# ScuffleCloud/SVT-AV1-mirror

Measured on AMD Instinct MI355X. Metric: open-loop ME 64x64 superblocks/sec + achieved HBM GB/s, 4K preset-8, higher is better.
Workload: dtype u8

## Files before the change

### svt-av1-mirror_amd/csrc/svtme_stages.hip

```cpp
#include <hip/hip_ext.h>
#include <cstdlib>
#include <type_traits>

#include "svtme_me_common.h"

extern "C" bool svtme_hme_rt(const svtme_controls *c);

namespace svtme {


#define STAGE_A_BUF_DW 1024
#define STAGE_B_BUF_DW 640

template <int ND, typename P>
__device__ __forceinline__ void rows_qsad(P rp, int bstride_dw, const uint8_t *src, int src_stride,
                                          int k0, int k1, uint32_t acc[4]) {
    constexpr int CH = 64 / ND;
    for (int kc = k0; kc < k1; kc += CH) {
        const int ke         = min(k1, kc + CH);
        unsigned long long a = 0;
#pragma unroll 2
        for (int k = kc; k < ke; k++) {
            const P rd         = rp + k * bstride_dw;
            const uint32_t *sd = (const uint32_t *)(src + k * src_stride);
// ... 2265 lines not shown
        const uint32_t d3 = __builtin_amdgcn_alignbyte(t5, t4.w, (uint32_t)sh);
#pragma unroll
        for (int j = 0; j < NT; j++) {
            const int r = k - j;
            if (r < 0 || r >= ROWS)
                continue;
            acc[j][0] = qsad64(pair(d0, d1), src[r][0], acc[j][0]);
            acc[j][0] = qsad64(pair(d1, d2), src[r][1], acc[j][0]);
            acc[j][1] = qsad64(pair(d1, d2), src[r][0], acc[j][1]);
            acc[j][1] = qsad64(pair(d2, d3), src[r][1], acc[j][1]);
        }
    }
#pragma unroll
    for (int j = 0; j < NT; j++)
        M.template add_quads<true>((uint32_t)acc[j][0], (uint32_t)(acc[j][0] >> 32), (uint32_t)acc[j][1],
                                   (uint32_t)(acc[j][1] >> 32), obase + (uint32_t)((c + NC * j) * 8), 0, 8, qb);
}

template <bool SUB>
__device__ __forceinline__ void fp_rows32_whole(PuMin<true> &M, const uint8_t *g, int sdw, int h, uint32_t obase,
                                                const uint32_t (&src)[SUB ? 4 : 8][2], int by, int bx) {
    g     = uni_ptr(g);
    sdw   = UNI(sdw);
    h     = UNI(h);
    obase = (uint32_t)UNI(obase);
    const uint32_t qb = PuMin<true>::quad_b_rows();
    const int sh      = (int)((uintptr_t)g & 3);
    const __amdgpu_buffer_rsrc_t rs = plane_rsrc(g - sh);
    const uint32_t lo = (uint32_t)((by * 8) * sdw + bx * 2) * 4u;
    if constexpr (SUB) {
        fp_whole_class<true, 2>(M, rs, lo, sdw, sh, qb, obase, 0, src);
        if (h == 4)
            fp_whole_class<true, 2>(M, rs, lo, sdw, sh, qb, obase, 1, src);
        else
            fp_whole_class<true, 1>(M, rs, lo, sdw, sh, qb, obase, 1, src);
    } else {
        fp_whole_class<false, 4>(M, rs, lo, sdw, sh, qb, obase, 0, src);
        fp_whole_class<false, 4>(M, rs, lo, sdw, sh, qb, obase, 4, src);
    }
}

template <bool SUB>
__device__ __forceinline__ uint32_t fp_probe32(PuMin<true> &M, const uint8_t *g, int sdw,
                                               const uint32_t (&src)[SUB ? 4 : 8][2], int by, int bx) {
    constexpr int ROWS = SUB ? 4 : 8, RSTEP = SUB ? 2 : 1;
    g         = uni_ptr(g);
    sdw       = UNI(sdw);
    const int sh = (int)((uintptr_t)g & 3);
    const __amdgpu_buffer_rsrc_t rs = plane_rsrc(g - sh);
    const uint32_t lo = (uint32_t)((by * 8) * sdw + bx * 2) * 4u;
    u32x4a4 d[ROWS];
#pragma unroll
    for (int rr = 0; rr < ROWS; rr++) d[rr] = bld4(rs, lo, (uint32_t)(rr * RSTEP * sdw) * 4u);
    uint32_t s8 = 0;
#pragma unroll
    for (int rr = 0; rr < ROWS; rr++) {
        s8 = __builtin_amdgcn_sad_u8(__builtin_amdgcn_alignbyte(d[rr].y, d[rr].x, (uint32_t)sh), src[rr][0], s8);
        s8 = __builtin_amdgcn_sad_u8(__builtin_amdgcn_alignbyte(d[rr].z, d[rr].y, (uint32_t)sh), src[rr][1], s8);
    }
    M.add_probe(s8);
    return SUB ? s8 << 1 : s8;
}

struct FpArea {
    int16_t xo, yo, w, h, xc, yc;
    bool probe;
};
template <typename Probe>
__device__ __forceinline__ FpArea fp_area(const DevJob &dj, const SbGeo &G, int s, uint32_t zz, uint32_t rdiv,
                                          int16_t sc_x, int16_t sc_y, Probe probe_var) {
    const svtme_job &job    = dj.job;
    const svtme_controls &c = job.ctrl;
    const int l = s >> 2, r = s & 3;
    const uint32_t ox = G.ox, oy = G.oy;
    const bool mctf   = SF(job, me_type) == SVTME_ME_MCTF;
    const DevPlane &C = dj.cur.lv[0];
    const DevPlane &P = dj.ref[l][r].lv[0];
    int16_t xc = sc_x, yc = sc_y;
    uint16_t dist = ref_dist_const(job, l, r);
    if (!mctf)
        dist = scaled_dist(dist);
    int16_t w = i16(min((int)(SF(c, me_sa.sa_min.width) * dist), (int)SF(c, me_sa.sa_max.width)));
    int16_t h = i16(min((int)(SF(c, me_sa.sa_min.height) * dist), (int)SF(c, me_sa.sa_max.height)));
    if (SF(c, mv_sa_adj_enabled) && (!SF(c, mv_sa_adj_nearest_ref_only) || r == 0)) {
        const int mth = (int)SF(c, mv_sa_adj_mv_size_th), mul = (int)SF(c, mv_sa_adj_sa_multiplier);
        if (absi(xc) > mth)
            w = i16(w * mul);
        if (absi(yc) > mth)
            h = i16(h * mul);
    }
    w = i16((max(1u, ((uint32_t)(int32_t)w / rdiv)) + 7) & ~0x07u);
    h = i16(max(3u, ((uint32_t)(int32_t)h / rdiv)));
    const int16_t pad = 63, org_x = (int16_t)ox, org_y = (int16_t)oy;
    if (c.me_early_exit_th) {
        if (zz < (c.me_early_exit_th / 6)) {
            w = 1;
            h = 1;
        }
    } else if ((xc != 0 || yc != 0) && SF(job, is_ref)) {
        const int16_t pw = i16(P.width), ph = i16(P.height);
        xc = ((org_x + xc) < -pad) ? i16(-pad - org_x) : xc;
        xc = ((org_x + xc) > pw - 1) ? i16(xc - ((org_x + xc) - (pw - 1))) : xc;
        yc = ((org_y + yc) < -pad) ? i16(-pad - org_y) : yc;
        yc = ((org_y + yc) > ph - 1) ? i16(yc - ((org_y + yc) - (ph - 1))) : yc;
        const uint8_t *cb = C.base + (ptrdiff_t)oy * C.stride + ox;
        const uint32_t zero_sad =
            wave_nxm(P.base + (ptrdiff_t)oy * P.stride + ox, 2 * P.stride, cb, 2 * C.stride, (int)(G.bh >> 1),
                     (int)G.bw)
            << 1;
        const uint32_t hme_mv_sad = wave_nxm(P.base + (ptrdiff_t)((int)oy + yc) * P.stride + ((int)ox + xc),
                                             2 * P.stride, cb, 2 * C.stride, (int)(G.bh >> 1), (int)G.bw)
            << 1;
        const uint64_t zc = (uint64_t)zero_sad << 8, hc = (uint64_t)hme_mv_sad << 8;
        if (min_u64(zc, hc) == zc) {
            xc = 0;
            yc = 0;
        }
    }
    const bool probe = SF(c, me_8x8_var_enabled) && (w * h > 24);
    if (probe) {
        const uint32_t var = probe_var(P.base + (ptrdiff_t)((int)oy + yc) * P.stride + ((int)ox + xc));
        if (var > c.me_sr_mult2_th) {
            w = i16((max(1, w * 3 / 2) + 7) & ~0x7);
            h = i16(max(1, h * 3 / 2));
        }
        if (var < c.me_sr_div4_th) {
            w = i16((max(1, w >> 2) + 7) & ~0x7);
            h = i16(max(1, h >> 2));
            h = i16(max(3, (int)h));
        } else if (var < c.me_sr_div2_th) {
            w = i16((min((int)w, w >> 1) + 7) & ~0x7);
            h = i16(min((int)h, h >> 1));
            h = i16(max(3, (int)h));
        }
    }
    const int16_t pic_w = (int16_t)job.width, pic_h = (int16_t)job.height;
    int16_t xo = i16(xc - (w >> 1));
    int16_t yo = i16(yc - (h >> 1));
    xo = ((org_x + xo) < -pad) ? i16(-pad - org_x) : xo;
    w  = ((org_x + xo) < -pad) ? i16(w - (-pad - (org_x + xo))) : w;
    xo = ((org_x + xo) > pic_w - 1) ? i16(xo - ((org_x + xo) - (pic_w - 1))) : xo;
    w  = ((org_x + xo + w) > pic_w) ? i16(max(1, w - ((org_x + xo + w) - pic_w))) : w;
    w  = (w < 8) ? w : i16(w & ~0x07);
    yo = ((org_y + yo) < -pad) ? i16(-pad - org_y) : yo;
    h  = ((org_y + yo) < -pad) ? i16(h - (-pad - (org_y + yo))) : h;
    yo = ((org_y + yo) > pic_h - 1) ? i16(yo - ((org_y + yo) - (pic_h - 1))) : yo;
    h  = (org_y + yo + h > pic_h) ? i16(max(1, h - ((org_y + yo + h) - pic_h))) : h;
    return FpArea{xo, yo, w, h, xc, yc, probe};
}

__device__ __forceinline__ bool direct_records(const DevJob &dj) {
    return SF(dj.job, me_type) == SVTME_ME_MCTF && dj.parts == 1 && dj.out_sb == nullptr;
}
__device__ __forceinline__ void direct_record(svtme_ref_record *rec, const CSlot &v, unsigned long long k8,
                                              unsigned long long k16, unsigned long long k32, unsigned long long k64) {
    const int lane   = threadIdx.x & 63;
    uint32_t *o      = (uint32_t *)rec;
    const uint32_t wm = magic_u32((uint32_t)max(1, (int)v.w));
    auto put = [&](unsigned long long key, int pu) {
        uint32_t sad = U32MAX, mv = 0;
        if (v.searched) {
            const uint32_t ord = (uint32_t)key;
            sad                = (uint32_t)(key >> 32);
            int16_t mx, my;
            if (v.probe && ord == 0) {
                mx = v.xc;
                my = v.yc;
            } else {
                const int p = (int)ord - (int)v.probe;
                const int q = mdiv(p, wm);
                my          = i16(v.yo + q);
                mx          = i16(v.xo + (p - q * v.w));
            }
            mv = ((uint32_t)(uint16_t)my << 16) | (uint16_t)mx;
        }
        o[pu]      = sad;
        o[85 + pu] = mv;
    };
    put(k8, 21 + lane);
    if ((lane & 3) == 0)
        put(k16, 5 + (lane >> 2));
    if ((lane & 15) == 0)
        put(k32, 1 + (lane >> 4));
    if (lane == 63)
        put(k64, 0);
    if (lane < 6) {
        const uint32_t t[6] = {(uint32_t)v.hme_sad, (uint32_t)(v.hme_sad >> 32),
                               (uint32_t)(uint16_t)v.sc_x | ((uint32_t)(uint16_t)v.sc_y << 16), v.zz,
                               (uint32_t)v.searched | ((uint32_t)v.do_ref << 8) | ((uint32_t)v.tf_exit << 16), 0u};
        o[170 + lane] = t[lane];
    }
}

__device__ __forceinline__ CSlot fp_unsearched(uint64_t hme_sad, uint32_t zz, int16_t sc_x, int16_t sc_y, uint8_t dref,
                                               uint8_t tf_exit) {
    return CSlot{hme_sad, zz, sc_x, sc_y, 0, 0, 0, 0, 0, 0, dref, 0, tf_exit};
}

template <bool SUB, bool K32, int TQ = (SUB ? FP_TQ : 2), bool WIDE = false, int WHOLE = 7>
__device__ __forceinline__ void fp_slot(const DevJob &dj, const SbGeo &G, int s, const uint32_t (&src)[SUB ? 4 : 8][2],
                                        int by, int bx, uint64_t hme_sad, uint32_t zz, uint32_t rdiv, int16_t sc_x,
                                        int16_t sc_y, uint8_t dref, uint8_t tf_exit, int part, uint32_t parts,
                                        unsigned long long *kp, CSlot *cs, svtme_ref_record *rec = nullptr) {
    const int lane = threadIdx.x & 63;
    const int l = s >> 2, r = s & 3;
    const uint32_t ox = G.ox, oy = G.oy;
    if (!dref || tf_exit) {
        const CSlot cv = fp_unsearched(hme_sad, zz, sc_x, sc_y, dref, tf_exit);
        if (part == 0 && lane == 0)
            *cs = cv;
        if (rec)
            direct_record(rec, cv, 0, 0, 0, 0);
        return;
    }
    const DevPlane &P = dj.ref[l][r].lv[0];
    PuMin<K32> M;
    M.clear();
    const FpArea A = fp_area(dj, G, s, zz, rdiv, sc_x, sc_y, [&](const uint8_t *g) {
        const int sh = (int)((uintptr_t)g & 3);
        uint32_t p8, p64;
        if constexpr (K32) {
            p8  = fp_probe32<SUB>(M, g, P.stride >> 2, src, by, bx);
            p64 = wave_sum_u32(p8);
        } else {
            fp_rows<SUB, K32, 1>(M, (const uint32_t *)(g - sh), P.stride >> 2, sh, 1, 1, 0, 1, 0u, src, by, bx);
            M.finalize();
            p8  = (uint32_t)(PuMin<K32>::template out<SUB>(M.b8, true) >> 32);
            p64 = rl32((uint32_t)(PuMin<K32>::template out<SUB>(M.b64, false) >> 32), 63);
        }
        const uint32_t mean = p64 / 64;
        const int32_t diff  = (int32_t)p8 - (int32_t)mean;
        return wave_sum_u32((uint32_t)(diff * diff)) / 64;
    });
    const int16_t xo = A.xo, yo = A.yo, w = A.w, h = A.h, xc = A.xc, yc = A.yc;
    const bool probe = A.probe;
    HME_SUB(22);

    const uint8_t *g = P.base + (ptrdiff_t)((int)oy + yo) * P.stride + ((int)ox + xo);
    const int sh     = (int)((uintptr_t)g & 3);
    const int nq     = (sh + w + 3) >> 2;
    const int y0 = (int)(((uint32_t)h * part) / parts), y1 = (int)(((uint32_t)h * (part + 1)) / parts);
    const uint32_t obase = probe ? 1u : 0u;
    if constexpr (K32) {
        const bool whole = !WIDE && w == 8 && parts == 1;
        if ((SUB ? (WHOLE & 2) && (h == 3 || h == 4) : (WHOLE & 1) && h == 8) && whole)
            fp_rows32_whole<SUB>(M, g, P.stride >> 2, h, obase, src, by, bx);
        else
            fp_rows32<SUB, WIDE ? 6 : 2>(M, g, P.stride >> 2, w, y0, y1, obase, src, by, bx);
    }
    else
        fp_rows<SUB, K32, TQ>(M, (const uint32_t *)(g - sh), P.stride >> 2, sh, w, nq, y0, y1, obase, src, by, bx);
    HME_SUB(23);
    M.finalize();
    const unsigned long long k8  = PuMin<K32>::template out<SUB>(M.b8, true);
    const unsigned long long k16 = PuMin<K32>::template out<SUB>(M.b16, false);
    const unsigned long long k32 = PuMin<K32>::template out<SUB>(M.b32, false);
    const unsigned long long k64 = PuMin<K32>::template out<SUB>(M.b64, false);
    if (parts == 1) {
        kp[21 + lane] = k8;
        if ((lane & 3) == 0)
            kp[5 + (lane >> 2)] = k16;
        if ((lane & 15) == 0)
            kp[1 + (lane >> 4)] = k32;
        if (lane == 63)
            kp[0] = k64;
    } else {
        atomicMin(&kp[21 + lane], k8);
        if ((lane & 3) == 0)
            atomicMin(&kp[5 + (lane >> 2)], k16);
        if ((lane & 15) == 0)
            atomicMin(&kp[1 + (lane >> 4)], k32);
        if (lane == 63)
            atomicMin(&kp[0], k64);
    }
    const CSlot cv{hme_sad, zz, sc_x, sc_y, xo, yo, w, xc, yc, 1, dref, (uint8_t)probe, 0};
    if (part == 0 && lane == 0)
        *cs = cv;
    if (rec)
        direct_record(rec, cv, k8, k16, k32, k64);
}


template <bool SUB, bool K32, bool WIDE = false>
__global__ void __launch_bounds__(256) __attribute__((amdgpu_waves_per_eu(SUB ? 5 : 4, 8))) k_stage_c1(const DevBatch B) {
    const int lane = threadIdx.x & 63, wid = threadIdx.x >> 6;
    const uint32_t u = UNI(xcd_remap(blockIdx.x, gridDim.x) * 4 + wid);
    if (u >= B.total)
        return;
    uint32_t gw;
    const DevJob &dj        = batch_job(B, u, &gw);
    const svtme_job &job    = dj.job;
    const uint32_t parts  = dj.parts;
    const uint32_t per_sb = dj.R * parts;
    const uint32_t sb_local = UNI(gw / per_sb);
    const uint32_t rem      = gw - sb_local * per_sb;
    const int k             = UNI(rem / parts);
    const int part          = UNI(rem - (uint32_t)k * parts);
    const int s             = k < job.num_refs[0] ? k : 4 + (k - job.num_refs[0]);
    const SbGeo G     = sb_geo(dj, sb_local);
    const uint32_t ox = G.ox, oy = G.oy;
    const bool mctf   = job.me_type == SVTME_ME_MCTF;
    constexpr int ROWS = SUB ? 4 : 8, RSTEP = SUB ? 2 : 1;
    const int z16 = lane >> 2, k4 = lane & 3;
    const int by  = ((z16 >> 3) << 2) | (((z16 >> 1) & 1) << 1) | (k4 >> 1);
    const int bx  = (((z16 >> 2) & 1) << 2) | ((z16 & 1) << 1) | (k4 & 1);

    const DevPlane &C = dj.cur.lv[0];
    uint32_t src[ROWS][2];
#pragma unroll
    for (int rr = 0; rr < ROWS; rr++) {
        const uint32_t *sp =
            (const uint32_t *)(C.base + (ptrdiff_t)(oy + by * 8 + rr * RSTEP) * C.stride + ox + bx * 8);
        src[rr][0] = sp[0];
        src[rr][1] = sp[1];
    }
    const SlotCentre scv   = final_centre(job, dj.bst + sb_local, valid_mask(job));
    const uint64_t hme_sad = rl64(scv.hme_sad, s);
    const uint32_t zz = rl32(scv.zz, s), rdiv = rl32(scv.reduce_div, s);
    const int16_t sc_x = (int16_t)rl32((uint32_t)(int32_t)scv.sc_x, s);
    const int16_t sc_y = (int16_t)rl32((uint32_t)(int32_t)scv.sc_y, s);
    const uint8_t dref = (uint8_t)rl32(scv.do_ref, s);
    const uint8_t tf_exit = mctf && rl64(scv.hme_sad, 0) < job.tf_me_exit_th;
    CSlot *cs = dj.cslot + (size_t)sb_local * dj.R + k;
    unsigned long long *kp = dj.keys + ((size_t)sb_local * dj.R + k) * SVTME_PU_COUNT;
    svtme_ref_record *rec = direct_records(dj) ? dj.out_records + (size_t)sb_local * dj.R + k : nullptr;
    fp_slot<SUB, K32, (SUB ? FP_TQ : 2), WIDE>(dj, G, s, src, by, bx, hme_sad, zz, rdiv, sc_x, sc_y, dref, tf_exit, part,
                                             parts, kp, cs, rec);
}

#define FPW_PITCH 80
#define FPW_BOFF 40
#define FPW_ROWS 96
#define FPW_TQ 4

struct FpW {
    uint32_t b8t, b8b, b16, b32, b64;
};

__device__ __forceinline__ uint32_t fpw_min_hr(uint32_t v) {
    return min_u32(v, (uint32_t)__builtin_amdgcn_update_dpp((int)v, (int)v, 0x128, 0xF, 0xF, false));
}

template <bool MASK, bool K8 = true>
__device__ __forceinline__ void fpw_pair(FpW &m, unsigned long long T, unsigned long long T2, unsigned long long Bq,
                                         unsigned long long B2, int e0, int ev, uint32_t sel16, uint32_t sel32,
                                         int p16, int p32) {
    const uint32_t tl = (uint32_t)T, th = (uint32_t)(T >> 32), tl2 = (uint32_t)T2, th2 = (uint32_t)(T2 >> 32);
    const uint32_t bl = (uint32_t)Bq, bh = (uint32_t)(Bq >> 32), bl2 = (uint32_t)B2, bh2 = (uint32_t)(B2 >> 32);
    auto k8 = [&](uint32_t v, int e) {
        const uint32_t k = (e & 1) ? ((v & 0xFFFF0000u) | (uint32_t)e) : ((v << 16) | (uint32_t)e);
        return (MASK && e >= ev) ? 0xFFFFFFFFu : k;
    };
    if constexpr (K8) {
        m.b8t = min_u32(min_u32(m.b8t, k8(tl, e0)), k8(tl, e0 + 1));
        m.b8t = min_u32(min_u32(m.b8t, k8(th, e0 + 2)), k8(th, e0 + 3));
        m.b8t = min_u32(min_u32(m.b8t, k8(tl2, e0 + 4)), k8(tl2, e0 + 5));
        m.b8t = min_u32(min_u32(m.b8t, k8(th2, e0 + 6)), k8(th2, e0 + 7));
        m.b8b = min_u32(min_u32(m.b8b, k8(bl, e0)), k8(bl, e0 + 1));
        m.b8b = min_u32(min_u32(m.b8b, k8(bh, e0 + 2)), k8(bh, e0 + 3));
        m.b8b = min_u32(min_u32(m.b8b, k8(bl2, e0 + 4)), k8(bl2, e0 + 5));
        m.b8b = min_u32(min_u32(m.b8b, k8(bh2, e0 + 6)), k8(bh2, e0 + 7));
    }
    const uint32_t sl = dpp_add<0xB1>(tl + bl), sh = dpp_add<0xB1>(th + bh);
    const uint32_t sl2 = dpp_add<0xB1>(tl2 + bl2), sh2 = dpp_add<0xB1>(th2 + bh2);
    auto k16 = [&](uint32_t v, int e) {
        const uint32_t k = __builtin_amdgcn_perm(v, (uint32_t)e, sel16);
        return (MASK && e + p16 >= ev) ? 0xFFFFFFFFu : k;
    };
    m.b16 = min_u32(min_u32(m.b16, k16(sl, e0)), k16(sh, e0 + 2));
    m.b16 = min_u32(min_u32(m.b16, k16(sl2, e0 + 4)), k16(sh2, e0 + 6));
    const uint32_t xl = dpp_add<0x4E>(sl), xh = dpp_add<0x4E>(sh);
    const uint32_t xl2 = dpp_add<0x4E>(sl2), xh2 = dpp_add<0x4E>(sh2);
    const uint32_t va = __builtin_amdgcn_perm(xh, xl, sel32), vb = __builtin_amdgcn_perm(xh2, xl2, sel32);
    const auto sw       = __builtin_amdgcn_permlane16_swap(va, vb, false, false);
    const uint32_t s32  = sw[0] + sw[1];
    const uint32_t k32  = (s32 << 12) | (uint32_t)e0;
    m.b32               = min_u32(m.b32, (MASK && e0 + p32 >= ev) ? 0xFFFFFFFFu : k32);
    const uint32_t s64h = dpp_add<0x141>(s32);
    const auto sw2      = __builtin_amdgcn_permlane32_swap(s64h, s64h, false, false);
    const uint32_t s64  = sw2[0] + sw2[1];
    const uint32_t k64  = (s64 << 12) | (uint32_t)e0;
    m.b64               = min_u32(m.b64, (MASK && e0 + p32 >= ev) ? 0xFFFFFFFFu : k64);
}

__device__ __forceinline__ uint32_t pk_min_u16(uint32_t a, uint32_t b) {
    typedef unsigned short u16x2 __attribute__((ext_vector_type(2)));
    return __builtin_bit_cast(uint32_t, __builtin_elementwise_min(__builtin_bit_cast(u16x2, a), __builtin_bit_cast(u16x2, b)));
}

__device__ __forceinline__ uint32_t fpw_rebase(uint32_t b, uint32_t m, uint32_t base) {
    return min_u32(b, m == 0xFFFFFFFFu ? m : m + base);
}

typedef uint32_t u32x2v __attribute__((ext_vector_type(2)));
struct FpwRow {
    u32x2v v[FPW_TQ + 1];
};
template <int OFF>
__device__ __forceinline__ u32x2v fpw_ds64(uint32_t a) {
    u32x2v r;
    asm volatile("ds_read_b64 %0, %1 offset:%2" : "=v"(r) : "v"(a), "i"(OFF));
    return r;
}
template <int G>
__device__ __forceinline__ void fpw_row_issue(FpwRow &R, uint32_t lb) {
    constexpr int ROW = (G / 4) * 8 + (G % 4) * 2, O = 4 * ROW * FPW_PITCH;
    R.v[0] = fpw_ds64<O>(lb);
    R.v[2] = fpw_ds64<O + 8>(lb);
    R.v[4] = fpw_ds64<O + 16>(lb);
    R.v[1] = fpw_ds64<O + 4 * FPW_BOFF>(lb);
// ... 723 lines not shown
            const uint32_t t = wave_sum_u32(sad);
            if (lane == 0)
                st.sum8[s] = t;
        }
        if (lane < 21)
            decode(lane, sad, mv);
    }
    __syncthreads();
    stage_c_tail<true, NW>(st, dj, sb_local, G.bw, G.bh, vmask);
}

__global__ void __launch_bounds__(256) __attribute__((amdgpu_waves_per_eu(4, 8))) k_stage_e(const DevBatch B) {
    __shared__ StC st;
    uint32_t sb_local;
    const DevJob &dj     = batch_job(B, xcd_remap(blockIdx.x, gridDim.x), &sb_local);
    const SbGeo G        = sb_geo(dj, sb_local);
    const uint32_t vmask = valid_mask(dj.job);
    stage_e_body(st, dj, sb_local, G, vmask, dj.cslot + (size_t)sb_local * dj.R,
                 dj.keys + (size_t)sb_local * dj.R * SVTME_PU_COUNT, dj.parts > 1);
}

struct HmeA {
    Dec d;
    unsigned long long key[SVTME_A_N];
    int16_t kxo[SVTME_A_N], kyo[SVTME_A_N];
    uint32_t need;
    HSrch srch[48];
    int32_t nsrch, nitems;
    int32_t nitems3, base2;
    int32_t end1, base3;
    unsigned long long key1[32];
    int16_t x1o[32], y1o[32];
    HSrch1 s1[32];
    int32_t nsrch1, nitems1;
    int16_t hx[32], hy[32];
    uint64_t hsad[32];
    __attribute__((aligned(16))) uint8_t src4[16][32];
    __attribute__((aligned(16))) uint8_t src1[32][HL2_PITCH];
};

template <int RND>
__device__ __forceinline__ void a1_table(HmeA &A, const DevJob &dj, uint32_t vmask, int16_t sox, int16_t soy, int kh,
                                         uint32_t l0need = 0, int16_t l00x = 0, int16_t l00y = 0,
                                         bool gate = false) {
    const svtme_job &job    = dj.job;
    const svtme_controls &c = job.ctrl;
    const int lane          = threadIdx.x & 63;
    const int s = lane / 6, k = lane - 6 * (lane / 6), l = s >> 2;
    bool on = lane < 48 && slot_valid(vmask, s) && tl_or_l0(job, l) &&
              (k < 2 ? c.prehme_enable != 0 : (c.enable_hme_flag && c.enable_hme_level0_flag));
    if (RND == 1)
        on = on && (k < 2 || s == 0);
    if (RND == 2)
        on = on && k >= 2 && s > 0 && ((l0need >> s) & 1u);
    bool mk    = false;
    int items3 = 0, items2 = 0;
    HSrch e;
    if (on) {
        const DevPlane &P = dj.ref[l][s & 3].lv[2];
        int16_t aw = k < 2 ? dj.ph_sa[s][k][0] : dj.l0_sa[s][0];
        int16_t ah = k < 2 ? dj.ph_sa[s][k][1] : dj.l0_sa[s][1];
        if (RND == 2)
            hme_l0_area(c, l, s & 3, dj.sdist[s], l00x, l00y, &aw, &ah);
        int16_t xo, yo, sw, shh;
        bool skip;
        if (k < 2) {
            prehme_area(P, sox, soy, aw, ah, &xo, &yo, &sw, &shh);
            skip   = c.prehme_skip_search_line != 0;
            e.id   = (uint8_t)(SVTME_A_PH + s * 2 + k);
            e.need = (uint8_t)(s * 2);
        } else {
            hme_l0_rect(c, P, sox, soy, aw, ah, (k - 2) >> 1, (k - 2) & 1, &xo, &yo, &sw, &shh);
            skip   = false;
            e.id   = (uint8_t)(SVTME_A_L0 + s * 4 + (k - 2));
            e.need = (uint8_t)(s * 2 + 1);
        }
        A.kxo[e.id]    = xo;
        A.kyo[e.id]    = yo;
        const int nrows = (sw > 0 && shh > 0) ? (skip ? shh / 2 : shh) : 0;
        if (nrows > 0) {
            const uint8_t *w0 = P.base + (ptrdiff_t)(soy + yo) * P.stride + (sox + xo);
            e.sh              = (uint8_t)((uintptr_t)w0 & 3);
            e.a0              = w0 - e.sh;
            e.sa_w            = sw;
            e.skip            = skip;
            const int nq      = (e.sh + sw + 3) >> 2;
            e.ncols           = (int16_t)((nq + HQ16 - 1) / HQ16);
            e.ncm             = magic_u32((uint32_t)e.ncols);
            if (skip) {
                e.cnt0  = (int16_t)nrows;
                e.cnt1  = 0;
                e.ylast = (int16_t)(2 * nrows - 1 + 2 * (kh - 1));
                items3  = e.ncols * ((nrows + HT16 - 1) / HT16);
                items2  = e.ncols * ((nrows + 1) / 2);
            } else {
                e.cnt0  = (int16_t)((nrows + 1) >> 1);
                e.cnt1  = (int16_t)(nrows >> 1);
                e.ylast = (int16_t)(nrows - 1 + 2 * (kh - 1));
                items3  = e.ncols * 2 * ((e.cnt0 + HT16 - 1) / HT16);
                items2  = e.ncols * 2 * ((e.cnt0 + 1) / 2);
            }
            mk = true;
        }
    }
    const bool l0    = k >= 2;
    const bool g     = RND == 0 && gate && mk && !l0 && l == 1;
    const int n3_pre = (int)wave_sum_u32(mk && !l0 && !g ? (uint32_t)items3 : 0u);
    const int n3_l0  = (int)wave_sum_u32(mk && l0 ? (uint32_t)items3 : 0u);
    const int n2_l0  = (int)wave_sum_u32(mk && l0 ? (uint32_t)items2 : 0u);
    const bool split = ((n3_pre + 63) / 64) * HT16 + ((n2_l0 + 63) / 64) * 2 < ((n3_pre + n3_l0 + 63) / 64) * HT16;
    const bool t2    = mk && split && l0;
    const int items  = t2 ? items2 : items3;
    e.tt             = (uint8_t)(t2 ? 2 : HT16);
    int n3s, n2s, ngs;
    const int k3 = wave_compact(mk && !t2 && !g, &n3s), k2 = wave_compact(t2, &n2s), kg = wave_compact(g, &ngs);
    const int i3 = wave_incl_scan(mk && !t2 && !g ? items : 0), i2 = wave_incl_scan(t2 ? items : 0);
    const int ig = wave_incl_scan(g ? items : 0);
    const int N3 = (int)lane63((uint32_t)i3), N2 = (int)lane63((uint32_t)i2), NG = (int)lane63((uint32_t)ig);
    const int base2 = (N3 + 63) & ~63;
    const int end1  = N2 ? base2 + N2 : N3;
    const int base3 = (end1 + 63) & ~63;
    if (mk) {
        e.item0 = g ? base3 + ig - items : t2 ? base2 + i2 - items : i3 - items;
        A.srch[g ? n3s + n2s + kg : t2 ? n3s + k2 : k3] = e;
    }
    if (lane == 0) {
        A.nsrch   = n3s + n2s + ngs;
        A.nitems3 = N3;
        A.base2   = base2;
        A.end1    = end1;
        A.base3   = NG ? base3 : end1;
        A.nitems  = NG ? base3 + NG : end1;
    }
}

__device__ __forceinline__ bool a1_mirrored(const HmeA &A, const svtme_controls &c, uint32_t need, int id) {
    const int r = ((id - SVTME_A_PH) >> 1) & 3, k = (id - SVTME_A_PH) & 1;
    if (c.me_early_exit_th && A.d.zz[r] < c.me_early_exit_th)
        return true;
    if (!((need >> (2 * r)) & 1u))
        return false;
    const int id0 = SVTME_A_PH + 2 * r + k;
    uint32_t best;
    int x, y;
    key_result(A.key[id0], &best, &x, &y);
    const uint32_t sad = best * 2;
    const int16_t col = i16((x + A.kxo[id0]) * 4), row = i16((y + A.kyo[id0]) * 4);
    return sad < 32 * 32 || (absi(col) < 16 && absi(row) < 16);
}

struct HmeSh {
    DevJob dj;
    BState bs;
    CSlot cin[8];
    SlotCentre cen[8];
    uint8_t tf_exit;
    union U {
        HmeA a;
        StC st;
    } u;
};

#define HME_PRIO_HI() __builtin_amdgcn_s_setprio(2)
#define HME_PRIO_LO() __builtin_amdgcn_s_setprio(0)
#define HME_WAVES_PER_EU 8
template <bool FP, bool SUB_ME, bool K32, bool RT = false, int NW = 4>
__global__ void __launch_bounds__(64 * NW) __attribute__((amdgpu_waves_per_eu(HME_WAVES_PER_EU, HME_WAVES_PER_EU))) k_hme(const DevBatch B) {
    static_assert(NW == 3 || NW == 4, "k_hme: 3 or 4 wavefronts");
    static_assert(sizeof(HmeSh) <= 16384, "HmeSh: ten workgroups per CU (160 KB of LDS)");
    constexpr int NT = 64 * NW;
    __shared__ HmeSh sh;
    const int tid = threadIdx.x, lane = tid & 63, wid = UNI(tid >> 6);
    uint32_t sb_local;
    const DevJob &gj = batch_job(B, xcd_remap(blockIdx.x, gridDim.x), &sb_local);
    {
        static_assert(sizeof(DevJob) % 16 == 0 && sizeof(DevJob) / 16 <= 2 * NT, "DevJob: at most two uint4 per thread");
        if (tid < (int)(sizeof(DevJob) / 16))
            ((uint4 *)&sh.dj)[tid] = ((const uint4 *)&gj)[tid];
        if (sizeof(DevJob) / 16 > NT && tid + NT < (int)(sizeof(DevJob) / 16))
            ((uint4 *)&sh.dj)[tid + NT] = ((const uint4 *)&gj)[tid + NT];
    }
    __syncthreads();
    const DevJob &dj        = sh.dj;
    const svtme_job &job    = dj.job;
    const svtme_controls &c = job.ctrl;
    const SbGeo G           = sb_geo(dj, sb_local);
    const uint32_t vmask    = valid_mask(job);
    Dec &d                  = sh.u.a.d;
    const int16_t sox = i16(((int16_t)G.ox) >> 2), soy = i16(((int16_t)G.oy) >> 2);
    const int kh  = (int)(G.bh >> 2) >> 1;
    const int kh1 = (int)(G.bh >> 2);
    const bool zz_on = c.me_early_exit_th || c.me_safe_limit_zz_th;
    HME_STAMP(0);

    if (wid == 0) {
        dec_init(d);
        uint32_t accv = 0;
        if (zz_on) {
            const int r = lane >> 1, h = lane & 1;
            const bool row_in = r < (int)(G.bh >> 1);
            const DevPlane &C = dj.cur.lv[0];
            u32x4a4 b0{}, b1{};
            if (row_in) {
                const uint32_t *cr = (const uint32_t *)(C.base + (ptrdiff_t)(G.oy + 2 * r) * C.stride + G.ox) + 8 * h;
                b0 = ldg4(cr), b1 = ldg4(cr + 4);
            }
            const uint8_t *fb[8];
            int fs[8];
#pragma unroll
            for (int sl = 0; sl < 8; sl++) {
                fb[sl] = gj.ref[sl >> 2][sl & 3].lv[0].base;
                fs[sl] = gj.ref[sl >> 2][sl & 3].lv[0].stride;
            }
            u32x4a4 a[8][2];
            bool sv[8];
            auto issue = [&](int sl) {
                sv[sl]    = slot_valid(vmask, sl) && tl_or_l0(job, sl >> 2);
                a[sl][0] = a[sl][1] = u32x4a4{};
                if (sv[sl] && row_in) {
                    const uint32_t *rr =
                        (const uint32_t *)(fb[sl] + (ptrdiff_t)(G.oy + 2 * r) * fs[sl] + G.ox) + 8 * h;
                    a[sl][0] = ldg4(rr), a[sl][1] = ldg4(rr + 4);
                }
            };
            auto sum = [&](int sl) {
                if (!sv[sl])
                    return;
                uint32_t acc = 0;
                if (row_in) {
                    acc = __builtin_amdgcn_sad_u8(a[sl][0].x, b0.x, acc);
                    acc = __builtin_amdgcn_sad_u8(a[sl][0].y, b0.y, acc);
                    acc = __builtin_amdgcn_sad_u8(a[sl][0].z, b0.z, acc);
                    acc = __builtin_amdgcn_sad_u8(a[sl][0].w, b0.w, acc);
                    acc = __builtin_amdgcn_sad_u8(a[sl][1].x, b1.x, acc);
                    acc = __builtin_amdgcn_sad_u8(a[sl][1].y, b1.y, acc);
                    acc = __builtin_amdgcn_sad_u8(a[sl][1].z, b1.z, acc);
                    acc = __builtin_amdgcn_sad_u8(a[sl][1].w, b1.w, acc);
                }
                const uint32_t t = wave_sum_u32(acc);
                accv             = lane == sl ? t : accv;
            };
            issue(0), issue(1), issue(2);
            issue(3), issue(4), issue(5);
            sum(0), sum(1), sum(2);
            issue(6), issue(7);
            sum(3), sum(4), sum(5);
            sum(6), sum(7);
        }
        HME_PRIO_HI();
        const uint32_t eet = c.me_early_exit_th, slz = c.me_safe_limit_zz_th;
        const uint32_t zth = c.zz_sad_th;
        const uint32_t zpct = c.zz_sad_pct;
        const int tli = job.temporal_layer_index, hl = job.hierarchical_levels, nl = job.num_lists;
        const bool sbr = job.similar_brightness_refs != 0;
        const uint32_t acc = accv;
        const bool have    = slot_valid(vmask, lane) && tl_or_l0(job, lane >> 2);
        uint32_t zz = U32MAX;
        bool dref   = true;
        if (eet || slz) {
            if (have) {
                zz                 = acc << 1;
                const uint32_t pix = G.bw * G.bh;
                zz                 = pix == 4096u ? (zz * 64 * 64) >> 12 : (zz * 64 * 64) / pix;
            }
            const uint32_t best = wave_min_u32(zz);
            if (have && (lane & 3) > 0 && tli > 0 && best < zth && (uint32_t)((zz - best) * 100u) > (uint32_t)(zpct * best))
                dref = false;
            if (slz) {
                const uint32_t z0 = rl32(zz, 0), z4 = rl32(zz, 4);
                const bool safe = hl > 0 && nl == 2 && tli >= hl && sbr && z0 < slz && z4 < slz;
                if (safe && slot_valid(vmask, lane) && (lane & 3) > 0)
                    dref = false;
            }
        }
        if (lane < 8) {
            d.zz[lane]     = zz;
            d.do_ref[lane] = dref ? 1 : 0;
        }
        const int s       = lane >> 1;
        const uint32_t zs = (uint32_t)__builtin_amdgcn_ds_bpermute(4 * s, (int)zz);
        const uint32_t ds = (uint32_t)__builtin_amdgcn_ds_bpermute(4 * s, dref ? 1 : 0);
        const bool act    = lane < 16 && slot_valid(vmask, s) && tl_or_l0(job, s >> 2) && ds;
        const bool nd     = act && ((lane & 1) ? !(eet && zs < (eet >> 2)) : !(eet && zs < eet));
        const unsigned long long m = __ballot(nd);
        if (lane == 0)
            sh.u.a.need = (uint32_t)m;
        HME_PRIO_LO();
    } else if (wid == 1) {
        if (lane < SVTME_A_N)
            sh.u.a.key[lane] = ~0ull;
        const bool gate = !RT && c.prehme_enable && c.prehme_l1_early_exit && job.num_lists == 2 &&
                          c.hme_search_method != SVTME_FULL_SAD_SEARCH && !(dj.paths & SVTME_PATH_NO_A1_GATE);
        a1_table<RT ? 1 : 0>(sh.u.a, dj, vmask, sox, soy, kh, 0, 0, 0, gate);
    } else {
        if (c.enable_hme_level2_flag) {
            const DevPlane &F = dj.cur.lv[0];
            constexpr int NP = 128 / (NT - 128);
            u32x4a4 v[NP];
#pragma unroll
            for (int p = 0; p < NP; p++) {
                const int i = tid - 128 + p * (NT - 128), row = i >> 2, part = i & 3;
                v[p] = ldg4((const uint32_t *)(F.base + (ptrdiff_t)(G.oy + 2 * row) * F.stride + G.ox + 16 * part));
            }
#pragma unroll
            for (int p = 0; p < NP; p++) {
                const int i = tid - 128 + p * (NT - 128), row = i >> 2, part = i & 3;
                ((uint4 *)sh.u.a.src1[row])[part] = make_uint4(v[p].x, v[p].y, v[p].z, v[p].w);
// ... 269 lines not shown
                        items             = e.ncols * shh;
                        mk                = true;
                    }
                }
            }
            sh.u.a.hx[lane]   = X;
            sh.u.a.hy[lane]   = Y;
            sh.u.a.hsad[lane] = SD;
        }
        int tot;
        const int kpos = wave_compact(mk, &tot);
        const int incl = wave_incl_scan(items);
        if (mk) {
            e.item0     = incl - items;
            sh.u.a.s1[kpos] = e;
        }
        if (lane == 63)
            sh.u.a.nitems1 = incl;
        if (lane == 0)
            sh.u.a.nsrch1 = tot;
    }
    __syncthreads();
    HME_PRIO_LO();
    HME_STAMP(4);
    {
        const int nlanes = 4 * sh.u.a.nitems1, nsrch = sh.u.a.nsrch1;
        const int pstride = dj.cur.lv[1].stride;
        auto tiles = [&](auto fullk) {
            for (int it4 = tid; it4 < nlanes; it4 += NT) {
                const int it    = it4 >> 2;
                const HSrch1 &e = sh.u.a.s1[find_search(sh.u.a.s1, nsrch, it)];
                const int local = it - e.item0;
                const int y = mdiv(local, e.ncm), col = local - y * e.ncols;
                const unsigned long long kk = hme_tile32q<decltype(fullk)::value>(e.a0, pstride, HQ1 * col, e.sh,
                                                                                  e.sa_w, y, kh1, sh.u.a.src4);
                if ((it4 & 3) == 0 && kk != ~0ull)
                    atomicMin(&sh.u.a.key1[e.id], kk);
            }
        };
        tiles(std::false_type());
    }
    __syncthreads();
    if (wid == 0 && lane < 32 && sh.u.a.hsad[lane] == ~0ull) {
        uint32_t best;
        int x, y;
        key_result(sh.u.a.key1[lane], &best, &x, &y);
        sh.u.a.hsad[lane] = hsub ? (uint64_t)best * 2 : best;
        sh.u.a.hx[lane]   = i16((x + sh.u.a.x1o[lane]) * 2);
        sh.u.a.hy[lane]   = i16((y + sh.u.a.y1o[lane]) * 2);
    }
    if (c.enable_hme_level2_flag) {
        if (wid == 0) {
            const int s = lane >> 2, l = s >> 2;
            bool mk   = false;
            int items = 0;
            HSrch1 e;
            if (lane < 32) {
                sh.u.a.key1[lane] = ~0ull;
                const bool listed = c.enable_hme_flag && slot_valid(vmask, s) && tl_or_l0(job, l);
                const bool keep   = c.prev_me_stage_based_exit_th &&
                                  sh.u.a.hsad[lane] < (c.prev_me_stage_based_exit_th >> 2);
                if (listed && !keep) {
                    const DevPlane &P = dj.ref[l][s & 3].lv[0];
                    int16_t xo, yo, sw, shh;
                    hme_refine_rect(2, P, (int16_t)G.ox, (int16_t)G.oy, (int16_t)c.hme_l2_sa.width,
                                    (int16_t)c.hme_l2_sa.height, sh.u.a.hx[lane], sh.u.a.hy[lane], &xo, &yo, &sw, &shh);
                    sh.u.a.x1o[lane]  = xo;
                    sh.u.a.y1o[lane]  = yo;
                    sh.u.a.hsad[lane] = ~0ull;
                    if (sw > 0 && shh > 0) {
                        const uint8_t *w0 = P.base + (ptrdiff_t)((int16_t)G.oy + yo) * P.stride + ((int16_t)G.ox + xo);
                        e.sh              = (uint8_t)((uintptr_t)w0 & 3);
                        e.a0              = w0 - e.sh;
                        e.sa_w            = sw;
                        e.ncols           = (int16_t)((((sw + 3) >> 2) + HQ - 1) / HQ);
                        e.ncm             = magic_u32((uint32_t)e.ncols);
                        e.id              = (uint8_t)lane;
                        items             = e.ncols * shh;
                        mk                = true;
                    }
                }
            }
            int tot;
            const int kpos = wave_compact(mk, &tot);
            const int incl = wave_incl_scan(items);
            if (mk) {
                e.item0            = incl - items;
                sh.u.a.s1[kpos] = e;
            }
            if (lane == 63)
                sh.u.a.nitems1 = incl;
            if (lane == 0)
                sh.u.a.nsrch1 = tot;
        }
        __syncthreads();
        {
            const int nlanes = 8 * sh.u.a.nitems1, nsrch = sh.u.a.nsrch1;
            const int pstride = dj.cur.lv[0].stride;
            const int kh2     = (int)(G.bh >> 1);
            for (int it8 = tid; it8 < nlanes; it8 += NT) {
                const int it    = it8 >> 3;
                const HSrch1 &e = sh.u.a.s1[find_search(sh.u.a.s1, nsrch, it)];
                const int local = it - e.item0;
                const int y = mdiv(local, e.ncm), col = local - y * e.ncols;
                const unsigned long long kk = hme_tile64(e.a0, pstride, HQ * col, e.sh, e.sa_w, y, kh2, sh.u.a.src1);
                if ((it8 & 7) == 0 && kk != ~0ull)
                    atomicMin(&sh.u.a.key1[e.id], kk);
            }
        }
        __syncthreads();
        if (wid == 0 && lane < 32 && sh.u.a.hsad[lane] == ~0ull) {
            uint32_t best;
            int x, y;
            key_result(sh.u.a.key1[lane], &best, &x, &y);
            sh.u.a.hsad[lane] = hsub ? (uint64_t)best * 2 : best;
            sh.u.a.hx[lane]   = i16(x + sh.u.a.x1o[lane]);
            sh.u.a.hy[lane]   = i16(y + sh.u.a.y1o[lane]);
        }
    }
    HME_STAMP(5);
    BState *b = FP ? &sh.bs : dj.bst + sb_local;
    if (wid == 0) {
        if (lane < 32) {
            b->hx[0][lane]         = sh.u.a.hx[lane];
            b->hy[0][lane]         = sh.u.a.hy[lane];
            b->hsad[0][lane]       = sh.u.a.hsad[lane];
            (&b->lx[0][0])[lane]   = (&d.lx[0][0])[lane];
            (&b->ly[0][0])[lane]   = (&d.ly[0][0])[lane];
            (&b->lsad[0][0])[lane] = (&d.lsad[0][0])[lane];
        }
        if (lane < 8) {
            b->zz[lane]     = d.zz[lane];
            b->do_ref[lane] = d.do_ref[lane];
        }
    }
    if (!FP) {
        HME_STAMP(6);
        return;
    }
    if (wid == 0) {
        HME_PRIO_HI();
        wave_lds_fence();
        const SlotCentre scv = final_centre(gj.job, &sh.bs, vmask);
        if (lane < 8)
            sh.cen[lane] = scv;
        if (lane == 0)
            sh.tf_exit = job.me_type == SVTME_ME_MCTF && scv.hme_sad < job.tf_me_exit_th;
    }
    __syncthreads();
    HME_PRIO_LO();
    HME_STOP(55);
    const int nrec = (int)dj.R, nr0 = (int)SF(gj.job, num_refs[0]);
    const uint8_t tfx = (uint8_t)UNI(sh.tf_exit);
    for (int k = 0, j = 0; k < nrec; k++) {
        constexpr int ROWS = SUB_ME ? 4 : 8, RSTEP = SUB_ME ? 2 : 1;
        const int s         = k < nr0 ? k : 4 + (k - nr0);
        const SlotCentre &v = sh.cen[s];
        const bool srch     = UNI(v.do_ref) && !tfx;
        const int owner     = srch ? j : NW - 1;
        j                   = srch ? (j + 1 == NW ? 0 : j + 1) : j;
        if (wid != owner)
            continue;
        if (!srch) {
            if (lane == 0)
                sh.cin[k] = fp_unsearched(v.hme_sad, v.zz, v.sc_x, v.sc_y, v.do_ref, tfx);
            continue;
        }
        int fl = lane;
        asm volatile("" : "+v"(fl));
        const int z16 = fl >> 2, k4 = fl & 3;
        const int by  = ((z16 >> 3) << 2) | (((z16 >> 1) & 1) << 1) | (k4 >> 1);
        const int bx  = (((z16 >> 2) & 1) << 2) | ((z16 & 1) << 1) | (k4 & 1);
        const DevPlane &C = gj.cur.lv[0];
        const int cst     = UNI(C.stride);
        const __amdgpu_buffer_rsrc_t crs = plane_rsrc(uni_ptr(C.base + (ptrdiff_t)G.oy * cst + G.ox));
        const uint32_t coff = (uint32_t)(by * 8 * cst + bx * 8);
        uint32_t src[ROWS][2];
#pragma unroll
        for (int rr = 0; rr < ROWS; rr++) {
            const auto v = __builtin_amdgcn_raw_buffer_load_b64(crs, (int)coff, rr * RSTEP * cst, 0);
            src[rr][0] = v[0];
            src[rr][1] = v[1];
        }
        fp_slot<SUB_ME, K32, 2, false, HME_WHOLE>(gj, G, s, src, by, bx, rl64(v.hme_sad, 0), (uint32_t)UNI(v.zz), (uint32_t)UNI(v.reduce_div),
                                (int16_t)UNI(v.sc_x), (int16_t)UNI(v.sc_y), (uint8_t)UNI(v.do_ref), tfx, 0, 1u,
                                &sh.u.st.keys[k][0], &sh.cin[k]);
    }
    HME_WAVE(1);
    __syncthreads();
    HME_STAMP(6);
    stage_e_body<NW>(sh.u.st, gj, sb_local, G, vmask, sh.cin, &sh.u.st.keys[0][0], false);
    HME_STAMP(7);
}

}

extern "C" void svtme_stage_a_list(const svtme_job *job, uint8_t *list, uint32_t *count) {
    const svtme_controls &c = job->ctrl;
    uint32_t n = 0;
    for (int s = 0; s < 8; s++) {
        const int l = s >> 2, r = s & 3;
        if (l >= job->num_lists || r >= job->num_refs[l])
            continue;
        if (!(job->temporal_layer_index > 0 || l == 0))
            continue;
        const bool zz = c.me_early_exit_th || c.me_safe_limit_zz_th;
        const bool l0 = c.enable_hme_flag && c.enable_hme_level0_flag;
        if (svtme_hme_rt(&c) && s > 0) {
            if (zz)
                list[n++] = (uint8_t)((TA_ZZ << 3) | s);
        } else if (zz || l0)
            list[n++] = (uint8_t)((TA_HME << 3) | s);
        if (c.prehme_enable)
            list[n++] = (uint8_t)((TA_PH << 3) | s);
    }
    *count = n;
}

extern "C" void svtme_stage_a1_list(const svtme_job *job, uint8_t *list, uint32_t *count) {
    const svtme_controls &c = job->ctrl;
    uint32_t n = 0;
    if (svtme_hme_rt(&c) && c.enable_hme_flag && c.enable_hme_level0_flag)
        for (int s = 1; s < 8; s++) {
            const int l = s >> 2, r = s & 3;
            if (l >= job->num_lists || r >= job->num_refs[l])
                continue;
            if (!(job->temporal_layer_index > 0 || l == 0))
                continue;
            list[n++] = (uint8_t)((TA_L0RT << 3) | s);
        }
    *count = n;
}

extern "C" void svtme_stage_b_list(const svtme_job *job, uint8_t *list, uint32_t *count) {
    const svtme_controls &c = job->ctrl;
    uint32_t n = 0;
    if (c.enable_hme_flag && (c.enable_hme_level1_flag || c.enable_hme_level2_flag))
        for (int s = 0; s < 8; s++) {
            const int l = s >> 2, r = s & 3;
            if (l >= job->num_lists || r >= job->num_refs[l])
                continue;
            if (!(job->temporal_layer_index > 0 || l == 0))
                continue;
            for (int q = 0; q < 4; q++) list[n++] = (uint8_t)((s << 2) | q);
        }
    *count = n;
}

static void fp_area_bound(const svtme_controls *c, uint32_t *w, uint32_t *h) {
    uint32_t mw = c->me_sa.sa_max.width, mh = c->me_sa.sa_max.height;
    if (c->mv_sa_adj_enabled) {
        mw *= c->mv_sa_adj_sa_multiplier;
        mh *= c->mv_sa_adj_sa_multiplier;
    }
    mw = (mw + 7) & ~7u;
    mh = mh < 3 ? 3 : mh;
    if (c->me_8x8_var_enabled && c->me_sr_mult2_th != 0xFFFFFFFFu) {
        mw = ((mw * 3 / 2) + 7) & ~7u;
        mh = mh * 3 / 2;
    }
    *w = mw;
    *h = mh;
}

extern "C" void svtme_hme_prepare(DevJob *dj) {
    const svtme_job &job    = dj->job;
    const svtme_controls &c = job.ctrl;
    for (int s = 0; s < 8; s++) {
        const int l = s >> 2, r = s & 3;
        const bool valid = l < job.num_lists && r < job.num_refs[l];
        const uint16_t dist = valid ? svtme::ref_dist_const(job, l, r) : 1;
        dj->sdist[s] = dist;
        int16_t w = 0, h = 0;
        if (valid)
            svtme::hme_l0_area(c, l, r, dist, 0, 0, &w, &h);
        dj->l0_sa[s][0] = w;
        dj->l0_sa[s][1] = h;
        const uint32_t f = svtme::scaled_dist(dist);
        for (int k = 0; k < 2; k++) {
            const uint32_t mw = (uint32_t)c.prehme_sa_cfg[k].sa_min.width * f, xw = c.prehme_sa_cfg[k].sa_max.width;
            const uint32_t mh = (uint32_t)c.prehme_sa_cfg[k].sa_min.height * f, xh = c.prehme_sa_cfg[k].sa_max.height;
            dj->ph_sa[s][k][0] = (int16_t)(uint16_t)(mw < xw ? mw : xw);
            dj->ph_sa[s][k][1] = (int16_t)(uint16_t)(mh < xh ? mh : xh);
        }
    }
}

extern "C" bool svtme_hme_fused(const svtme_job *job) {
    const svtme_controls &c = job->ctrl;
    return (job->width % 64) == 0 && c.hme_search_method != SVTME_FULL_SAD_SEARCH;
}
static bool hme_fused(const DevJob &dj) { return svtme_hme_fused(&dj.job) && !(dj.paths & SVTME_PATH_NO_FUSED_HME); }

extern "C" uint32_t svtme_hme_waves(const svtme_job *job) {
    const svtme_controls &c = job->ctrl;
    uint32_t R = 0;
    for (int l = 0; l < job->num_lists && l < 2; l++) R += job->num_refs[l];
    return c.me_search_method != SVTME_FULL_SAD_SEARCH && !svtme_hme_rt(&c) && R <= 4 ? 3u : 4u;
}
extern "C" uint32_t svtme_hme_waves_paths(const svtme_job *job, uint32_t paths) {
    return (paths & SVTME_PATH_HME_4WAVES) ? 4u : svtme_hme_waves(job);
}
static uint32_t hme_waves(const DevJob &dj) {
    const bool whole = svtme_hme_fused(&dj.job) && dj.parts == 1 &&
                       !(dj.paths & (SVTME_PATH_NO_FUSED_HME | SVTME_PATH_SPLIT_PASS));
    return whole ? svtme_hme_waves_paths(&dj.job, dj.paths) : 4u;
}

extern "C" bool svtme_hme_rt(const svtme_controls *c) {
    return c->enable_me_sr_adjustment && c->distance_based_hme_resizing && c->reduce_hme_l0_sr_th_min &&
           c->reduce_hme_l0_sr_th_max;
}

extern "C" bool svtme_l1_full(const svtme_controls *c) {
    return c->hme_search_method == SVTME_FULL_SAD_SEARCH && c->enable_hme_flag && c->enable_hme_level1_flag &&
           !c->enable_hme_level2_flag && c->hme_l1_sa.width <= 16 && c->hme_l1_sa.height <= 16;
}
static bool l1_full(const DevJob &dj) { return svtme_l1_full(&dj.job.ctrl) && !(dj.paths & SVTME_PATH_NO_L1_FULL); }

extern "C" bool svtme_l0_full(const DevJob *dj) {
    const svtme_controls &c = dj->job.ctrl;
    if (c.hme_search_method != SVTME_FULL_SAD_SEARCH || c.prehme_enable || !c.enable_hme_flag ||
        !c.enable_hme_level0_flag || svtme_hme_rt(&c) || (dj->job.width % 64) % 16 != 0 ||
        (dj->paths & SVTME_PATH_NO_L0_FULL))
        return false;
    for (int s = 0; s < 8; s++)
        if (dj->l0_sa[s][0] > 16 || dj->l0_sa[s][1] > 16)
            return false;
    return true;
}

extern "C" bool svtme_l0_full_job(const svtme_job *job) {
    DevJob dj{};
    dj.job = *job;
    svtme_hme_prepare(&dj);
    return svtme_l0_full(&dj);
}

static bool l0_full_short(const DevJob *dj) {
    for (int s = 0; s < 8; s++)
        if (dj->l0_sa[s][1] > 8)
            return false;
    return true;
}
// ... 200 lines not shown
```

Before: 73.08 million.

## Decode full-pel keys into local records per wave, use stage-C tail

In the fused HME kernel, each wave that runs the full-pel search now decodes its PU keys directly into per-slot SAD/MV records and summary fields in shared memory, instead of writing raw keys and CSlot headers for the later stage_e_body pass. Unused slots are initialised by the last wave, and the epilogue calls stage_c_tail on these records. The aim is to drop the separate key decode and reduction pass and shrink the shared struct by removing cin. In exchange, each searching wave does more work (divisions, a wave sum) before the barrier, and correctness depends on stage_c_tail matching the old stage_e semantics.

```diff
diff --git a/svt-av1-mirror_amd/csrc/svtme_stages.hip b/svt-av1-mirror_amd/csrc/svtme_stages.hip
--- a/svt-av1-mirror_amd/csrc/svtme_stages.hip
+++ b/svt-av1-mirror_amd/csrc/svtme_stages.hip
@@ -2441,28 +2441,32 @@
 __device__ __forceinline__ bool direct_records(const DevJob &dj) {
     return SF(dj.job, me_type) == SVTME_ME_MCTF && dj.parts == 1 && dj.out_sb == nullptr;
 }
+__device__ __forceinline__ void key_decode(const CSlot &v, uint32_t wm, unsigned long long key, uint32_t &sad, uint32_t &mv) {
+    sad = U32MAX, mv = 0;
+    if (v.searched) {
+        const uint32_t ord = (uint32_t)key;
+        sad                = (uint32_t)(key >> 32);
+        int16_t mx, my;
+        if (v.probe && ord == 0) {
+            mx = v.xc;
+            my = v.yc;
+        } else {
+            const int p = (int)ord - (int)v.probe;
+            const int q = mdiv(p, wm);
+            my          = i16(v.yo + q);
+            mx          = i16(v.xo + (p - q * v.w));
+        }
+        mv = ((uint32_t)(uint16_t)my << 16) | (uint16_t)mx;
+    }
+}
 __device__ __forceinline__ void direct_record(svtme_ref_record *rec, const CSlot &v, unsigned long long k8,
                                               unsigned long long k16, unsigned long long k32, unsigned long long k64) {
     const int lane   = threadIdx.x & 63;
     uint32_t *o      = (uint32_t *)rec;
     const uint32_t wm = magic_u32((uint32_t)max(1, (int)v.w));
     auto put = [&](unsigned long long key, int pu) {
-        uint32_t sad = U32MAX, mv = 0;
-        if (v.searched) {
-            const uint32_t ord = (uint32_t)key;
-            sad                = (uint32_t)(key >> 32);
-            int16_t mx, my;
-            if (v.probe && ord == 0) {
-                mx = v.xc;
-                my = v.yc;
-            } else {
-                const int p = (int)ord - (int)v.probe;
-                const int q = mdiv(p, wm);
-                my          = i16(v.yo + q);
-                mx          = i16(v.xo + (p - q * v.w));
-            }
-            mv = ((uint32_t)(uint16_t)my << 16) | (uint16_t)mx;
-        }
+        uint32_t sad, mv;
+        key_decode(v, wm, key, sad, mv);
         o[pu]      = sad;
         o[85 + pu] = mv;
     };
@@ -2481,21 +2485,57 @@
     }
 }
 
+__device__ __forceinline__ void local_record(StC &st, int s, const CSlot &v, unsigned long long k8, unsigned long long k16,
+                                             unsigned long long k32, unsigned long long k64) {
+    const int lane    = threadIdx.x & 63;
+    uint32_t *o       = st.rec[s];
+    const uint32_t wm = magic_u32((uint32_t)max(1, (int)v.w));
+    auto put = [&](unsigned long long key, int pu) {
+        uint32_t sad, mv;
+        key_decode(v, wm, key, sad, mv);
+        o[pu]      = sad;
+        o[85 + pu] = mv;
+        return sad;
+    };
+    const uint32_t sad8 = put(k8, 21 + lane);
+    if ((lane & 3) == 0)
+        put(k16, 5 + (lane >> 2));
+    if ((lane & 15) == 0)
+        put(k32, 1 + (lane >> 4));
+    if (lane == 63)
+        put(k64, 0);
+    const uint32_t sum8 = v.searched ? wave_sum_u32(sad8) : 0u;
+    if (lane == 0) {
+        st.hme_sad[s]  = v.hme_sad;
+        st.zz[s]       = v.zz;
+        st.sc_x[s]     = v.sc_x;
+        st.sc_y[s]     = v.sc_y;
+        st.searched[s] = v.searched;
+        st.do_ref[s]   = v.do_ref;
+        st.sum8[s]     = sum8;
+    }
+}
+
 __device__ __forceinline__ CSlot fp_unsearched(uint64_t hme_sad, uint32_t zz, int16_t sc_x, int16_t sc_y, uint8_t dref,
                                                uint8_t tf_exit) {
     return CSlot{hme_sad, zz, sc_x, sc_y, 0, 0, 0, 0, 0, 0, dref, 0, tf_exit};
 }
 
-template <bool SUB, bool K32, int TQ = (SUB ? FP_TQ : 2), bool WIDE = false, int WHOLE = 7>
+template <bool SUB, bool K32, int TQ = (SUB ? FP_TQ : 2), bool WIDE = false, int WHOLE = 7, bool LREC = false>
 __device__ __forceinline__ void fp_slot(const DevJob &dj, const SbGeo &G, int s, const uint32_t (&src)[SUB ? 4 : 8][2],
                                         int by, int bx, uint64_t hme_sad, uint32_t zz, uint32_t rdiv, int16_t sc_x,
                                         int16_t sc_y, uint8_t dref, uint8_t tf_exit, int part, uint32_t parts,
-                                        unsigned long long *kp, CSlot *cs, svtme_ref_record *rec = nullptr) {
+                                        unsigned long long *kp, CSlot *cs, svtme_ref_record *rec = nullptr,
+                                        StC *lst = nullptr) {
     const int lane = threadIdx.x & 63;
     const int l = s >> 2, r = s & 3;
     const uint32_t ox = G.ox, oy = G.oy;
     if (!dref || tf_exit) {
         const CSlot cv = fp_unsearched(hme_sad, zz, sc_x, sc_y, dref, tf_exit);
+        if constexpr (LREC) {
+            local_record(*lst, s, cv, 0, 0, 0, 0);
+            return;
+        }
         if (part == 0 && lane == 0)
             *cs = cv;
         if (rec)
@@ -2545,6 +2585,11 @@
     const unsigned long long k16 = PuMin<K32>::template out<SUB>(M.b16, false);
     const unsigned long long k32 = PuMin<K32>::template out<SUB>(M.b32, false);
     const unsigned long long k64 = PuMin<K32>::template out<SUB>(M.b64, false);
+    if constexpr (LREC) {
+        const CSlot cv{hme_sad, zz, sc_x, sc_y, xo, yo, w, xc, yc, 1, dref, (uint8_t)probe, 0};
+        local_record(*lst, s, cv, k8, k16, k32, k64);
+        return;
+    }
     if (parts == 1) {
         kp[21 + lane] = k8;
         if ((lane & 3) == 0)
@@ -3574,7 +3619,6 @@
 struct HmeSh {
     DevJob dj;
     BState bs;
-    CSlot cin[8];
     SlotCentre cen[8];
     uint8_t tf_exit;
     union U {
@@ -4150,6 +4194,20 @@
     HME_STOP(55);
     const int nrec = (int)dj.R, nr0 = (int)SF(gj.job, num_refs[0]);
     const uint8_t tfx = (uint8_t)UNI(sh.tf_exit);
+    if (wid == NW - 1) {
+        StC &st = sh.u.st;
+        if (lane < 8 && !(lane < 4 ? lane < nr0 : nr0 + (lane - 4) < nrec)) {
+            st.hme_sad[lane]  = U32MAX;
+            st.zz[lane]       = U32MAX;
+            st.sc_x[lane]     = 0;
+            st.sc_y[lane]     = 0;
+            st.searched[lane] = 0;
+            st.do_ref[lane]   = 0;
+            st.sum8[lane]     = 0;
+        }
+        if (lane == 0)
+            st.tf_exit = nrec > 0 ? tfx : 0;
+    }
     for (int k = 0, j = 0; k < nrec; k++) {
         constexpr int ROWS = SUB_ME ? 4 : 8, RSTEP = SUB_ME ? 2 : 1;
         const int s         = k < nr0 ? k : 4 + (k - nr0);
@@ -4160,8 +4218,7 @@
         if (wid != owner)
             continue;
         if (!srch) {
-            if (lane == 0)
-                sh.cin[k] = fp_unsearched(v.hme_sad, v.zz, v.sc_x, v.sc_y, v.do_ref, tfx);
+            local_record(sh.u.st, s, fp_unsearched(v.hme_sad, v.zz, v.sc_x, v.sc_y, v.do_ref, tfx), 0, 0, 0, 0);
             continue;
         }
         int fl = lane;
@@ -4180,14 +4237,14 @@
             src[rr][0] = v[0];
             src[rr][1] = v[1];
         }
-        fp_slot<SUB_ME, K32, 2, false, HME_WHOLE>(gj, G, s, src, by, bx, rl64(v.hme_sad, 0), (uint32_t)UNI(v.zz), (uint32_t)UNI(v.reduce_div),
+        fp_slot<SUB_ME, K32, 2, false, HME_WHOLE, true>(gj, G, s, src, by, bx, rl64(v.hme_sad, 0), (uint32_t)UNI(v.zz), (uint32_t)UNI(v.reduce_div),
                                 (int16_t)UNI(v.sc_x), (int16_t)UNI(v.sc_y), (uint8_t)UNI(v.do_ref), tfx, 0, 1u,
-                                &sh.u.st.keys[k][0], &sh.cin[k]);
+                                nullptr, nullptr, nullptr, &sh.u.st);
     }
     HME_WAVE(1);
     __syncthreads();
     HME_STAMP(6);
-    stage_e_body<NW>(sh.u.st, gj, sb_local, G, vmask, sh.cin, &sh.u.st.keys[0][0], false);
+    stage_c_tail<true, NW>(sh.u.st, gj, sb_local, G.bw, G.bh, vmask);
     HME_STAMP(7);
 }
 
```

Result: no change. 72.74 million (-0.5%).
